# coqui-ai/TTS

Measured on NVIDIA H100. Metric: audio_samples_per_sec, higher is better.
Workload: dtype f32

## Files before the change

### tts_b200/csrc/conv_tc.cuh

```cuda
#pragma once
#include <cuda_runtime.h>
#include <stdint.h>

namespace b200tts {
namespace tc {

enum : int { PREC_FP32 = 0, PREC_BF16 = 1, PREC_FP16 = 2, PREC_F16X3 = 4 };
enum : int { ERR_RANGE = 1 };
constexpr float F16X3_MAX = 65504.f;
constexpr uint32_t SPIN_LIMIT = 1u << 22;

__device__ __forceinline__ uint32_t smem_u32(const void* p) { return (uint32_t)__cvta_generic_to_shared(p); }

__device__ __forceinline__ void mbar_init(uint32_t bar, uint32_t count) {
    asm volatile("mbarrier.init.shared::cta.b64 [%0], %1;" ::"r"(bar), "r"(count));
}
__device__ __forceinline__ void mbar_arrive(uint32_t bar) {
    asm volatile("mbarrier.arrive.shared::cta.b64 _, [%0];" ::"r"(bar) : "memory");
}
__device__ __forceinline__ void mbar_expect_tx(uint32_t bar, uint32_t bytes) {
    asm volatile("mbarrier.arrive.expect_tx.shared::cta.b64 _, [%0], %1;" ::"r"(bar), "r"(bytes) : "memory");
}
__device__ __forceinline__ bool mbar_wait(uint32_t bar, uint32_t parity, int* err) {
#pragma unroll 1
    for (uint32_t i = 0; i < SPIN_LIMIT; ++i) {
        uint32_t ok;
        asm volatile("{\n.reg .pred p;\nmbarrier.try_wait.parity.shared::cta.b64 p, [%1], %2;\nselp.u32 %0, 1, 0, p;\n}"
                     : "=r"(ok) : "r"(bar), "r"(parity) : "memory");
        if (ok) return true;
    }
    if (err) { *reinterpret_cast<volatile int*>(err) = 1; __threadfence_system(); }
    return false;
}
__device__ __forceinline__ void bulk_g2s(uint32_t dst, const void* src, uint32_t bytes, uint32_t bar) {
    asm volatile("cp.async.bulk.shared::cluster.global.mbarrier::complete_tx::bytes [%0], [%1], %2, [%3];"
                 ::"r"(dst), "l"(src), "r"(bytes), "r"(bar) : "memory");
}
__device__ __forceinline__ void fence_async_smem() { asm volatile("fence.proxy.async.shared::cta;" ::: "memory"); }

__device__ __forceinline__ uint64_t make_desc(uint32_t saddr, uint32_t lbo_bytes) {
    uint64_t d = 0;
    d |= (uint64_t)((saddr >> 4) & 0x3FFF);
    d |= (uint64_t)((lbo_bytes >> 4) & 0x3FFF) << 16;
    d |= (uint64_t)((128u >> 4) & 0x3FFF) << 32;
    return d;
}

__device__ __forceinline__ void wgmma_fence() { asm volatile("wgmma.fence.sync.aligned;" ::: "memory"); }
__device__ __forceinline__ void wgmma_commit() { asm volatile("wgmma.commit_group.sync.aligned;" ::: "memory"); }
template <int N>
__device__ __forceinline__ void wgmma_wait() { asm volatile("wgmma.wait_group.sync.aligned %0;" ::"n"(N) : "memory"); }

#define B200_WGMMA_D128                                                                                                       \
    "{%0,%1,%2,%3,%4,%5,%6,%7,%8,%9,%10,%11,%12,%13,%14,%15,%16,%17,%18,%19,%20,%21,%22,%23,%24,%25,%26,%27,%28,%29,%30,%31,"    \
    "%32,%33,%34,%35,%36,%37,%38,%39,%40,%41,%42,%43,%44,%45,%46,%47,%48,%49,%50,%51,%52,%53,%54,%55,%56,%57,%58,%59,%60,%61,%62,%63," \
    "%64,%65,%66,%67,%68,%69,%70,%71,%72,%73,%74,%75,%76,%77,%78,%79,%80,%81,%82,%83,%84,%85,%86,%87,%88,%89,%90,%91,%92,%93,%94,%95," \
    "%96,%97,%98,%99,%100,%101,%102,%103,%104,%105,%106,%107,%108,%109,%110,%111,%112,%113,%114,%115,%116,%117,%118,%119,%120,%121,%122,%123,%124,%125,%126,%127},"
#define B200_WGMMA_D128_OPS(d)                                                                                                \
    "+f"(d[0]), "+f"(d[1]), "+f"(d[2]), "+f"(d[3]), "+f"(d[4]), "+f"(d[5]), "+f"(d[6]), "+f"(d[7]),                          \
    "+f"(d[8]), "+f"(d[9]), "+f"(d[10]), "+f"(d[11]), "+f"(d[12]), "+f"(d[13]), "+f"(d[14]), "+f"(d[15]),                    \
    "+f"(d[16]), "+f"(d[17]), "+f"(d[18]), "+f"(d[19]), "+f"(d[20]), "+f"(d[21]), "+f"(d[22]), "+f"(d[23]),                  \
    "+f"(d[24]), "+f"(d[25]), "+f"(d[26]), "+f"(d[27]), "+f"(d[28]), "+f"(d[29]), "+f"(d[30]), "+f"(d[31]),                  \
    "+f"(d[32]), "+f"(d[33]), "+f"(d[34]), "+f"(d[35]), "+f"(d[36]), "+f"(d[37]), "+f"(d[38]), "+f"(d[39]),                  \
    "+f"(d[40]), "+f"(d[41]), "+f"(d[42]), "+f"(d[43]), "+f"(d[44]), "+f"(d[45]), "+f"(d[46]), "+f"(d[47]),                  \
    "+f"(d[48]), "+f"(d[49]), "+f"(d[50]), "+f"(d[51]), "+f"(d[52]), "+f"(d[53]), "+f"(d[54]), "+f"(d[55]),                  \
    "+f"(d[56]), "+f"(d[57]), "+f"(d[58]), "+f"(d[59]), "+f"(d[60]), "+f"(d[61]), "+f"(d[62]), "+f"(d[63]),                  \
    "+f"(d[64]), "+f"(d[65]), "+f"(d[66]), "+f"(d[67]), "+f"(d[68]), "+f"(d[69]), "+f"(d[70]), "+f"(d[71]),                  \
    "+f"(d[72]), "+f"(d[73]), "+f"(d[74]), "+f"(d[75]), "+f"(d[76]), "+f"(d[77]), "+f"(d[78]), "+f"(d[79]),                  \
    "+f"(d[80]), "+f"(d[81]), "+f"(d[82]), "+f"(d[83]), "+f"(d[84]), "+f"(d[85]), "+f"(d[86]), "+f"(d[87]),                  \
    "+f"(d[88]), "+f"(d[89]), "+f"(d[90]), "+f"(d[91]), "+f"(d[92]), "+f"(d[93]), "+f"(d[94]), "+f"(d[95]),                  \
    "+f"(d[96]), "+f"(d[97]), "+f"(d[98]), "+f"(d[99]), "+f"(d[100]), "+f"(d[101]), "+f"(d[102]), "+f"(d[103]),              \
    "+f"(d[104]), "+f"(d[105]), "+f"(d[106]), "+f"(d[107]), "+f"(d[108]), "+f"(d[109]), "+f"(d[110]), "+f"(d[111]),          \
    "+f"(d[112]), "+f"(d[113]), "+f"(d[114]), "+f"(d[115]), "+f"(d[116]), "+f"(d[117]), "+f"(d[118]), "+f"(d[119]),          \
    "+f"(d[120]), "+f"(d[121]), "+f"(d[122]), "+f"(d[123]), "+f"(d[124]), "+f"(d[125]), "+f"(d[126]), "+f"(d[127])

__device__ __forceinline__ void wgmma_tf32_m64n256(float* d, uint64_t adesc, uint64_t bdesc, uint32_t acc) {
    asm volatile(
        "{\n.reg .pred p;\nsetp.ne.b32 p, %130, 0;\n"
        "wgmma.mma_async.sync.aligned.m64n256k8.f32.tf32.tf32 " B200_WGMMA_D128
        " %128, %129, p, 1, 1;\n}"
        : B200_WGMMA_D128_OPS(d)
        : "l"(adesc), "l"(bdesc), "r"(acc)
        : "memory");
}

__device__ __forceinline__ void wgmma_bf16_m64n256(float* d, uint64_t adesc, uint64_t bdesc, uint32_t acc) {
    asm volatile(
        "{\n.reg .pred p;\nsetp.ne.b32 p, %130, 0;\n"
        "wgmma.mma_async.sync.aligned.m64n256k16.f32.bf16.bf16 " B200_WGMMA_D128
        " %128, %129, p, 1, 1, 0, 0;\n}"
        : B200_WGMMA_D128_OPS(d)
        : "l"(adesc), "l"(bdesc), "r"(acc)
        : "memory");
}
__device__ __forceinline__ void wgmma_f16_m64n256(float* d, uint64_t adesc, uint64_t bdesc, uint32_t acc) {
    asm volatile(
        "{\n.reg .pred p;\nsetp.ne.b32 p, %130, 0;\n"
        "wgmma.mma_async.sync.aligned.m64n256k16.f32.f16.f16 " B200_WGMMA_D128
        " %128, %129, p, 1, 1, 0, 0;\n}"
        : B200_WGMMA_D128_OPS(d)
        : "l"(adesc), "l"(bdesc), "r"(acc)
        : "memory");
}
__device__ __forceinline__ void wgmma_f16_m64n256_rs(float* d, const uint32_t (&a)[4], uint64_t bdesc, uint32_t acc) {
    asm volatile(
        "{\n.reg .pred p;\nsetp.ne.b32 p, %133, 0;\n"
        "wgmma.mma_async.sync.aligned.m64n256k16.f32.f16.f16 " B200_WGMMA_D128
        " {%128, %129, %130, %131}, %132, p, 1, 1, 0;\n}"
        : B200_WGMMA_D128_OPS(d)
        : "r"(a[0]), "r"(a[1]), "r"(a[2]), "r"(a[3]), "l"(bdesc), "r"(acc)
        : "memory");
}

__device__ __forceinline__ void ldsm_x4(uint32_t (&r)[4], uint32_t addr) {
    asm volatile("ldmatrix.sync.aligned.m8n8.x4.shared.b16 {%0, %1, %2, %3}, [%4];"
                 : "=r"(r[0]), "=r"(r[1]), "=r"(r[2]), "=r"(r[3]) : "r"(addr) : "memory");
}
__device__ __forceinline__ uint32_t f16x2_times_2m11(uint32_t v) {
    uint32_t r;
    asm("mul.rn.f16x2 %0, %1, %2;" : "=r"(r) : "r"(v), "r"(0x10001000u));
    return r;
}

__device__ __forceinline__ uint32_t cvt_bf16x2(float lo, float hi) {
    uint32_t r;
    asm("cvt.rn.bf16x2.f32 %0, %1, %2;" : "=r"(r) : "f"(hi), "f"(lo));
    return r;
}
__device__ __forceinline__ uint32_t cvt_f16x2(float lo, float hi) {
    uint32_t r;
    asm("cvt.rn.f16x2.f32 %0, %1, %2;" : "=r"(r) : "f"(hi), "f"(lo));
    return r;
}
__device__ __forceinline__ void split_f16x2(float a, float b, uint32_t& hi, uint32_t& lo) {
    hi = cvt_f16x2(a, b);
    float ha, hb;
    asm("{\n.reg .b16 l, h;\nmov.b32 {l, h}, %2;\ncvt.f32.f16 %0, l;\ncvt.f32.f16 %1, h;\n}" : "=f"(ha), "=f"(hb) : "r"(hi));
    lo = cvt_f16x2((a - ha) * 2048.f, (b - hb) * 2048.f);
}

}
}
```

### tts_b200/csrc/conv_tc3.cuh

```cuda
#pragma once
#include <cuda_runtime.h>
#include <stdint.h>

#include "conv_tc.cuh"

namespace b200tts {
namespace tc3 {

using namespace tc;

constexpr int TT2 = 256;
constexpr int MROWS = 128;
constexpr int KC2 = 8;
constexpr int KC16 = 16;
constexpr int RAWS = 324;
constexpr int NRAW = 3;
constexpr int NA2 = 2;
constexpr int NB2 = 3;
constexpr int ACC_LD = 260;
constexpr int ACC_BYTES = MROWS * ACC_LD * 4;
constexpr int NPW = 3;
constexpr int NPROD = 32 * NPW;
constexpr int NCONS = 256;
constexpr int W_PROD = 8, W_LOAD = 8 + NPW;
constexpr int NTHREADS2 = 32 * (W_LOAD + 1);

struct Tc3Args {
    const float* x; long long x_bs; int x_cs; int Tin;
    float in_slope;
    const void* w;
    const float* rscale;
    const float* bias;
    const float* cond; long long cond_bs;
    int Cin, K, dil, pad, Rows, N;
    float* y; long long y_bs; int y_cs; int Tout;
    int ups;
    int Tq;
    const float* res; long long res_bs; int res_cs;
    const float* ymask; long long ymask_bs;
    float scale; float post_div; int relu; int accum; int mask_post;
    int mask_pre;
    int gate;
    int split;
    float* y2; long long y2_bs; int y2_cs; int accum2;
    int KJ;
    int dil_blk;
    int tstep;
    int rows_pad;
    int raw_w;
    int B, n_ttiles, n_rtiles;
    int* err;
    const int* lens; int rate_q, need_q, rate_in, need_in;
    int pref_off;
    int q_lo, q_hi, in_lo, t_lo;
    int near_src; float near_scale;
    const float* film; long long film_bs; int film_cs, film_half;
    const float* act_add; int lrelu; float act_param;
};

__device__ __forceinline__ int near_col(int t, int src, int dst, float scale) {
    if (dst == src) return t;
    if (dst == 2 * src) return t >> 1;
    return min((int)floorf(__fmul_rn((float)t, scale)), src - 1);
}

static inline size_t smem_bytes3(int rows_pad, int prec = PREC_FP32) {
    const bool b16 = prec == PREC_BF16 || prec == PREC_FP16;
    const size_t raw_ch = b16 ? KC16 : KC2, nsl = b16 ? 2 : 4;
    return (size_t)NRAW * raw_ch * RAWS * 4 + (size_t)NA2 * (nsl * rows_pad * 16) + NB2 * (nsl * MROWS * 16) + ACC_BYTES + 512;
}
static inline size_t ragged_table_bytes(int B) { return ((size_t)(B + 1) * sizeof(int) + 15) / 16 * 16; }

__device__ __forceinline__ void cp_async16(uint32_t dst, const void* src) {
    asm volatile("cp.async.cg.shared.global [%0], [%1], 16;" ::"r"(dst), "l"(src) : "memory");
}
__device__ __forceinline__ void cp_async16_zfill(uint32_t dst, const void* src, uint32_t src_bytes) {
    asm volatile("cp.async.cg.shared.global [%0], [%1], 16, %2;" ::"r"(dst), "l"(src), "r"(src_bytes) : "memory");
}
__device__ __forceinline__ void cp_async4_zfill(uint32_t dst, const void* src, uint32_t src_bytes) {
    asm volatile("cp.async.ca.shared.global [%0], [%1], 4, %2;" ::"r"(dst), "l"(src), "r"(src_bytes) : "memory");
}
__device__ __forceinline__ void named_bar_sync(int id, int n) { asm volatile("bar.sync %0, %1;" ::"r"(id), "r"(n) : "memory"); }
__device__ __forceinline__ void acc_ld16(const float* p, float* v) {
#pragma unroll
    for (int j = 0; j < 4; ++j) {
        const float4 t = *reinterpret_cast<const float4*>(p + 4 * j);
        v[4 * j] = t.x; v[4 * j + 1] = t.y; v[4 * j + 2] = t.z; v[4 * j + 3] = t.w;
    }
}

constexpr int TSTEP_GROUPED = 240;

template <bool HR, bool HA, bool SC>
__device__ __forceinline__ void lean_tile(const float* at, const float* bias, const float* rscale, const float* cond, int lane,
                                          const float* rq, float* yq, long long rcs, long long ycs, int row0, int Rows,
                                          bool do_st) {
    const int r8 = lane & 7, p4 = lane >> 3;
    const float* rrow[4];
    float* yrow[4];
    bool st_ok[4];
    float bv[4], sv[4];
#pragma unroll
    for (int i = 0; i < 4; ++i) {
        const int ri = row0 + 8 * i + r8, rci = ri < Rows ? ri : Rows - 1;
        rrow[i] = rq + (long long)rci * rcs + 4 * p4;
        yrow[i] = yq + (long long)rci * ycs + 4 * p4;
        st_ok[i] = do_st && ri < Rows;
        bv[i] = bias[rci];
        if (cond) bv[i] += __ldg(cond + rci);
        sv[i] = SC ? rscale[rci] : 1.f;
    }
    const float* ap = at + r8 * ACC_LD + 4 * p4;
    float r0[16], r1[16];
    auto pf = [&](int cg, float* r_) {
        if constexpr (HR) {
#pragma unroll
            for (int i = 0; i < 4; ++i)
                asm volatile("ld.global.v4.f32 {%0,%1,%2,%3}, [%4];" : "=f"(r_[4 * i]), "=f"(r_[4 * i + 1]), "=f"(r_[4 * i + 2]), "=f"(r_[4 * i + 3]) : "l"(rrow[i] + cg));
        }
    };
    auto group = [&](int cg, const float* rv, float* rn) {
        float o[16];
        if (cg + 16 < 128) pf(cg + 16, rn);
        if constexpr (HA) {
#pragma unroll
            for (int i = 0; i < 4; ++i)
                asm volatile("ld.global.v4.f32 {%0,%1,%2,%3}, [%4];" : "=f"(o[4 * i]), "=f"(o[4 * i + 1]), "=f"(o[4 * i + 2]), "=f"(o[4 * i + 3]) : "l"(yrow[i] + cg));
        }
#pragma unroll
        for (int i = 0; i < 4; ++i) {
            float4 t = *reinterpret_cast<const float4*>(ap + 8 * i * ACC_LD + cg);
            if constexpr (SC) { t.x *= sv[i]; t.y *= sv[i]; t.z *= sv[i]; t.w *= sv[i]; }
            t.x += bv[i]; t.y += bv[i]; t.z += bv[i]; t.w += bv[i];
            if constexpr (HR) { t.x += rv[4 * i]; t.y += rv[4 * i + 1]; t.z += rv[4 * i + 2]; t.w += rv[4 * i + 3]; }
            if constexpr (HA) { t.x += o[4 * i]; t.y += o[4 * i + 1]; t.z += o[4 * i + 2]; t.w += o[4 * i + 3]; }
            if (st_ok[i]) *reinterpret_cast<float4*>(yrow[i] + cg) = t;
        }
    };
    pf(0, r0);
#pragma unroll 1
    for (int cg = 0; cg < 128; cg += 32) {
        group(cg, r0, r1);
        group(cg + 16, r1, r0);
    }
}

template <bool SC, bool WG = false>
__device__ __forceinline__ void general_tile_body(const Tc3Args& a, const float* arow, int b, int rt, int q0, int lq, int half,
                                                  int lane) {
    const int ups = a.ups;
    const int r = rt * MROWS + lq * 32 + lane;
    const bool rok = r < a.Rows;
    const int rc = rok ? r : a.Rows - 1;
    const int qb = q0 + half * 128;
    float bias = a.bias[rc];
    if (a.cond) bias += __ldg(a.cond + (long long)b * a.cond_bs + rc);
    const float rs = SC ? a.rscale[rc] : 1.f;
    auto acc_ld = [&](const float* p, float* v) {
        acc_ld16(p, v);
        if constexpr (SC) {
#pragma unroll
            for (int i = 0; i < 16; ++i) v[i] *= rs;
        }
    };
    if constexpr (WG) {
        if (!rok) return;
        const long long rcs = (long long)rc;
        float* yrow = a.y + (long long)b * a.y_bs + rcs * a.y_cs;
        float* y2row = a.y2 ? a.y2 + (long long)b * a.y2_bs + rcs * a.y2_cs : nullptr;
        const float* rrow = a.res ? a.res + (long long)b * a.res_bs + rcs * a.res_cs : nullptr;
        const float* srow = a.film ? a.film + (long long)b * a.film_bs + rcs * a.film_cs : nullptr;
        const float* crow = srow ? srow + (long long)a.film_half * a.film_cs : nullptr;
        const float add = a.act_add ? __ldg(a.act_add + b) : 0.f;
        const bool has_add = a.act_add != nullptr, lrelu = a.lrelu != 0;
        const float slope = a.act_param;
        const bool vec_ok = ((reinterpret_cast<uintptr_t>(yrow) | reinterpret_cast<uintptr_t>(y2row) |
                              reinterpret_cast<uintptr_t>(rrow) | reinterpret_cast<uintptr_t>(srow) |
                              reinterpret_cast<uintptr_t>(crow)) & 15) == 0;
        for (int cg = 0; cg < 128; cg += 16) {
            float v[16];
            acc_ld(arow + cg, v);
#pragma unroll
            for (int j = 0; j < 4; ++j) {
                const int qq = qb + cg + 4 * j;
                if (qq >= a.Tout) break;
                const bool vec = vec_ok && qq + 3 < a.Tout;
                float r4[4] = {0.f, 0.f, 0.f, 0.f}, s4[4] = {0.f, 0.f, 0.f, 0.f}, c4[4] = {1.f, 1.f, 1.f, 1.f};
                if (vec) {
                    if (rrow) { const float4 t = *reinterpret_cast<const float4*>(rrow + qq); r4[0] = t.x; r4[1] = t.y; r4[2] = t.z; r4[3] = t.w; }
                    if (srow) {
                        const float4 t = *reinterpret_cast<const float4*>(srow + qq); s4[0] = t.x; s4[1] = t.y; s4[2] = t.z; s4[3] = t.w;
                        const float4 u = *reinterpret_cast<const float4*>(crow + qq); c4[0] = u.x; c4[1] = u.y; c4[2] = u.z; c4[3] = u.w;
                    }
                } else {
#pragma unroll
                    for (int e = 0; e < 4; ++e) {
                        const int qe = min(qq + e, a.Tout - 1);
                        if (rrow) r4[e] = rrow[qe];
                        if (srow) { s4[e] = srow[qe]; c4[e] = crow[qe]; }
                    }
                }
                float o[4], p[4];
#pragma unroll
                for (int e = 0; e < 4; ++e) {
                    float u = __fadd_rn(v[4 * j + e], bias);
                    if (lrelu) u = u > 0.f ? u : __fmul_rn(u, slope);
                    if (has_add) u = __fadd_rn(u, add);
                    if (rrow) u = __fadd_rn(u, r4[e]);
                    p[e] = u;
                    o[e] = srow ? __fadd_rn(s4[e], __fmul_rn(c4[e], u)) : u;
                }
                if (vec) {
                    if (y2row) *reinterpret_cast<float4*>(y2row + qq) = make_float4(p[0], p[1], p[2], p[3]);
                    *reinterpret_cast<float4*>(yrow + qq) = make_float4(o[0], o[1], o[2], o[3]);
                } else {
#pragma unroll
                    for (int e = 0; e < 4; ++e)
                        if (qq + e < a.Tout) {
                            if (y2row) y2row[qq + e] = p[e];
                            yrow[qq + e] = o[e];
                        }
                }
            }
        }
        return;
    }
    if (a.gate) {
        float* yrow = a.y + (long long)b * a.y_bs + (long long)(rc >> 1) * a.y_cs;
        const bool vec_ok = ((a.y_cs & 3) == 0) && ((reinterpret_cast<uintptr_t>(yrow) & 15) == 0);
        const bool even = (lane & 1) == 0;
        for (int cg = 0; cg < 128; cg += 16) {
            float v[16];
            acc_ld(arow + cg, v);
            const int q = qb + cg;
#pragma unroll
            for (int i = 0; i < 16; ++i) {
                const float u = v[i] + bias;
                const float act = even ? tanhf(u) : 1.f / (1.f + expf(-u));
                const float other = __shfl_xor_sync(0xffffffffu, act, 1);
                v[i] = act * other;
            }
            if (rok && even) {
#pragma unroll
                for (int j = 0; j < 4; ++j) {
                    const int qq = q + 4 * j;
                    if (vec_ok && qq + 3 < a.Tout) *reinterpret_cast<float4*>(yrow + qq) = make_float4(v[4 * j], v[4 * j + 1], v[4 * j + 2], v[4 * j + 3]);
                    else {
#pragma unroll
                        for (int e = 0; e < 4; ++e) if (qq + e < a.Tout) yrow[qq + e] = v[4 * j + e];
                    }
                }
            }
        }
    } else if (ups == 1) {
        float* yrow = a.y + (long long)b * a.y_bs + (long long)rc * a.y_cs;
        bool acc_r = a.accum != 0, mpost_r = a.mask_post != 0;
        if (a.split > 0) {
            if (rc < a.split) { acc_r = true; mpost_r = true; }
            else { yrow = a.y2 + (long long)b * a.y2_bs + (long long)(rc - a.split) * a.y2_cs; acc_r = a.accum2 != 0; mpost_r = false; }
        }
        const float* rrow = a.res ? a.res + (long long)b * a.res_bs + (long long)rc * a.res_cs : nullptr;
        const float* mrow = a.ymask ? a.ymask + (long long)b * a.ymask_bs : nullptr;
        const int ycs_eff = (a.split > 0 && rc >= a.split) ? a.y2_cs : a.y_cs;
        const bool vec_ok = ((ycs_eff & 3) == 0) && (!a.res || (a.res_cs & 3) == 0) &&
                            ((reinterpret_cast<uintptr_t>(yrow) & 15) == 0) &&
                            (!rrow || (reinterpret_cast<uintptr_t>(rrow) & 15) == 0);
        float rA[16], oA[16], rB[16], oB[16];
        auto prefetch = [&](int cg, float* r_, float* o_) {
            const int q = qb + cg;
#pragma unroll
            for (int j = 0; j < 4; ++j) {
                const int qq = q + 4 * j;
                if (vec_ok && qq + 3 < a.Tout) {
                    if (rrow) asm volatile("ld.global.v4.f32 {%0,%1,%2,%3}, [%4];" : "=f"(r_[4 * j]), "=f"(r_[4 * j + 1]), "=f"(r_[4 * j + 2]), "=f"(r_[4 * j + 3]) : "l"(rrow + qq));
                    if (acc_r) asm volatile("ld.global.v4.f32 {%0,%1,%2,%3}, [%4];" : "=f"(o_[4 * j]), "=f"(o_[4 * j + 1]), "=f"(o_[4 * j + 2]), "=f"(o_[4 * j + 3]) : "l"(yrow + qq));
                } else {
#pragma unroll
                    for (int e = 0; e < 4; ++e) {
                        const int qe = min(qq + e, a.Tout - 1);
                        if (rrow) asm volatile("ld.global.f32 %0, [%1];" : "=f"(r_[4 * j + e]) : "l"(rrow + qe));
                        if (acc_r) asm volatile("ld.global.f32 %0, [%1];" : "=f"(o_[4 * j + e]) : "l"(yrow + qe));
                    }
                }
            }
        };
        auto group = [&](int cg, const float* rv, const float* ov, float* rn, float* on) {
            float v[16];
            if (rok && cg + 16 < 128) prefetch(cg + 16, rn, on);
            acc_ld(arow + cg, v);
            const int q = qb + cg;
#pragma unroll
            for (int i = 0; i < 16; ++i) {
                float u = v[i] + bias;
                if (a.relu) u = fmaxf(u, 0.f);
                const float mk = mrow ? __ldg(mrow + min(q + i, a.Tout - 1)) : 1.f;
                if (a.mask_pre) u *= mk;
                if (a.res) u += rv[i];
                u *= a.scale;
                if (acc_r) u += ov[i];
                if (a.post_div != 1.f) u = u / a.post_div;
                if (mpost_r) u *= mk;
                v[i] = u;
            }
            if (rok) {
#pragma unroll
                for (int j = 0; j < 4; ++j) {
                    const int qq = q + 4 * j;
                    if (vec_ok && qq + 3 < a.Tout) {
                        *reinterpret_cast<float4*>(yrow + qq) = make_float4(v[4 * j], v[4 * j + 1], v[4 * j + 2], v[4 * j + 3]);
                    } else {
#pragma unroll
                        for (int e = 0; e < 4; ++e) if (qq + e < a.Tout) yrow[qq + e] = v[4 * j + e];
                    }
                }
            }
        };
        if (rok) prefetch(0, rA, oA);
#pragma unroll 1
        for (int cg = 0; cg < 128; cg += 32) {
            group(cg, rA, oA, rB, oB);
            group(cg + 16, rB, oB, rA, oA);
        }
    } else {
        if (!rok) return;
        const int co = rc / ups, ph = rc - co * ups;
        float* yrow = a.y + (long long)b * a.y_bs + (long long)co * a.y_cs + ph;
        for (int cg = 0; cg < 128; cg += 16) {
            float v[16];
            acc_ld(arow + cg, v);
#pragma unroll
            for (int i = 0; i < 16; ++i) {
                const int q = qb + cg + i;
                float u = v[i] + bias;
                if (a.relu) u = fmaxf(u, 0.f);
                const long long t = (long long)q * ups;
                if (q < a.Tq && t + ph < a.Tout) yrow[t] = u;
            }
        }
    }
}

template <bool SC>
__device__ __noinline__ void general_tile_call(const Tc3Args& a_ref, const float* arow, int b, int rt, int q0, int lq, int half,
                                               int lane) {
    const Tc3Args a = a_ref;
    general_tile_body<SC>(a, arow, b, rt, q0, lq, half, lane);
}

template <int GRP, bool SC>
__device__ __forceinline__ void grouped_tile(const Tc3Args& a, const float* accs, int b, int q0, int lq, int half, int lane) {
    constexpr int CH = 128 / GRP;
    constexpr int NQ = CH / 32;
    constexpr int NV = 4 * NQ;
    const int tq = lq * 32 + lane;
    const int co = (tq * NQ) >> 2;
    const int coff = 4 * ((tq & (4 / NQ - 1)) * NQ);
    const int cbeg = half ? 128 : 0;
    const int cend = half ? a.tstep : min(128, a.tstep);
    const bool has_res = a.res != nullptr, acc_r = a.accum != 0;
    const bool vec_ok = ((a.y_cs & 3) == 0) && ((a.y_bs & 3) == 0) && ((reinterpret_cast<uintptr_t>(a.y) & 15) == 0) &&
                        (!a.res || (((a.res_cs & 3) == 0) && ((a.res_bs & 3) == 0) && ((reinterpret_cast<uintptr_t>(a.res) & 15) == 0)));
    const bool fast = vec_ok && (q0 + a.tstep <= a.Tout);
    const float* rrow = has_res ? a.res + (long long)b * a.res_bs + (long long)co * a.res_cs : nullptr;
    float* yrow = a.y + (long long)b * a.y_bs + (long long)co * a.y_cs;
    float bias = a.bias[co];
    if (a.cond) bias += __ldg(a.cond + (long long)b * a.cond_bs + co);
    const float rs = SC ? a.rscale[co] : 1.f;
    auto load = [&](const float* rr, int q, float* dst) {
#pragma unroll
        for (int j = 0; j < NQ; ++j) {
            const int qq = q + 4 * j;
            if (fast || (vec_ok && qq + 3 < a.Tout)) {
                const float4 t = *reinterpret_cast<const float4*>(rr + qq);
                dst[4 * j] = t.x; dst[4 * j + 1] = t.y; dst[4 * j + 2] = t.z; dst[4 * j + 3] = t.w;
            } else {
#pragma unroll
                for (int e = 0; e < 4; ++e) dst[4 * j + e] = rr[min(qq + e, a.Tout - 1)];
            }
        }
    };
#pragma unroll 1
    for (int cg = cbeg; cg < cend; cg += 16) {
        float R[NV], rv[NV], ov[NV];
        if (has_res) load(rrow, q0 + cg + coff, rv);
        if (acc_r) load(yrow, q0 + cg + coff, ov);
        const float* p = accs + co * ACC_LD + cg + coff;
#pragma unroll
        for (int i = 0; i < NV; ++i) {
            const float p0 = p[i], p1 = p[CH * ACC_LD + a.dil + i];
            float s = p0 + p1;
            if constexpr (GRP == 4) s += p[2 * CH * ACC_LD + 2 * a.dil + i] + p[3 * CH * ACC_LD + 3 * a.dil + i];
            if constexpr (SC) s *= rs;
            R[i] = s;
        }
#pragma unroll
        for (int i = 0; i < NV; ++i) {
            float u = R[i] + bias;
            if (a.relu) u = fmaxf(u, 0.f);
            if (has_res) u += rv[i];
            u *= a.scale;
            if (acc_r) u += ov[i];
            if (a.post_div != 1.f) u = u / a.post_div;
            R[i] = u;
        }
        const int q = q0 + cg + coff;
#pragma unroll
        for (int j = 0; j < NQ; ++j) {
            const int qq = q + 4 * j;
            if (fast || (vec_ok && qq + 3 < a.Tout)) {
                *reinterpret_cast<float4*>(yrow + qq) = make_float4(R[4 * j], R[4 * j + 1], R[4 * j + 2], R[4 * j + 3]);
            } else {
#pragma unroll
                for (int e = 0; e < 4; ++e) if (qq + e < a.Tout) yrow[qq + e] = R[4 * j + e];
            }
        }
    }
}

template <int GRP, bool LEAN = true, int PREC = PREC_FP32, bool REFL = false, bool NEAR = false, bool WG = false>
__device__ __forceinline__ void tc3_body(const Tc3Args& a) {
    extern __shared__ __align__(128) unsigned char smem[];
    constexpr bool X3 = PREC == PREC_F16X3;
    constexpr bool B16 = PREC == PREC_BF16 || PREC == PREC_FP16;
    constexpr int KCH = PREC != PREC_FP32 ? KC16 : KC2;
    constexpr int RCH = B16 ? KC16 : KC2;
    constexpr int SPC = KCH / RCH;
    constexpr int NSL = B16 ? 2 : 4;
    constexpr int SLC = PREC != PREC_FP32 ? 8 : 4;
    constexpr int NB = NB2;
    constexpr bool SC = X3;
    const int tid = threadIdx.x, warp = tid >> 5, lane = tid & 31;
    const int ROWS = a.rows_pad, RAWW = a.raw_w, K = a.KJ;
    const uint32_t rawStage = (uint32_t)RCH * RAWS * 4;
    const uint32_t slabA = (uint32_t)ROWS * 16, stageA = NSL * slabA;
    const uint32_t slabB = (uint32_t)MROWS * 16, stageB = NSL * slabB;
    unsigned char* smRaw = smem;
    unsigned char* smA = smRaw + NRAW * rawStage;
    unsigned char* smB = smA + NA2 * stageA;
    float* accs = reinterpret_cast<float*>(smB + NB * stageB);
    uint64_t* bars = reinterpret_cast<uint64_t*>(reinterpret_cast<unsigned char*>(accs) + ACC_BYTES);
    const int A_FULL = 0, A_EMPTY = NA2, B_FULL = 2 * NA2, B_EMPTY = 2 * NA2 + NB;
    const uint32_t bar0 = smem_u32(bars);
    auto BAR = [&](int i) { return bar0 + 8u * (uint32_t)i; };

    const int nchunks = (a.Cin + KCH - 1) / KCH;
    const bool ragged = a.lens != nullptr;
    int* pref = reinterpret_cast<int*>(smem + a.pref_off);
    if (ragged) {
        for (int b = tid; b < a.B; b += NTHREADS2) {
            const long long e = (long long)a.lens[b] * a.rate_q + a.need_q;
            const int ext = (int)(e < (long long)a.Tq ? (e > 0 ? e : 0) : (long long)a.Tq);
            const int t_hi = (min(ext, a.q_hi) + a.tstep - 1) / a.tstep;
            pref[b + 1] = max(0, t_hi - a.t_lo) * a.n_rtiles;
        }
        __syncthreads();
        if (warp == 0) {
            const int per = (a.B + 31) / 32, lo = lane * per, hi = min(a.B, lo + per);
            int sum = 0;
            for (int b = lo; b < hi; ++b) sum += pref[b + 1];
            int incl = sum;
#pragma unroll
            for (int o = 1; o < 32; o <<= 1) { const int n = __shfl_up_sync(0xffffffffu, incl, o); if (lane >= o) incl += n; }
            int run = incl - sum;
            for (int b = lo; b < hi; ++b) { const int c = pref[b + 1]; pref[b + 1] = run + c; run += c; }
            if (lane == 0) pref[0] = 0;
        }
        __syncthreads();
    }
    const int tiles_total = ragged ? pref[a.B] : a.B * a.n_rtiles * a.n_ttiles;
    const int my_tiles = (tiles_total > (int)blockIdx.x) ? (tiles_total - 1 - (int)blockIdx.x) / (int)gridDim.x + 1 : 0;

    if (tid == 0) {
        for (int i = 0; i < NA2; ++i) { mbar_init(BAR(A_FULL + i), NPW); mbar_init(BAR(A_EMPTY + i), NCONS / 32); }
        for (int i = 0; i < NB; ++i) { mbar_init(BAR(B_FULL + i), 1); mbar_init(BAR(B_EMPTY + i), NCONS / 32); }
        asm volatile("fence.mbarrier_init.release.cluster;" ::: "memory");
    }
    __syncthreads();
    asm volatile("griddepcontrol.launch_dependents;" ::: "memory");
    if (warp != W_LOAD) asm volatile("griddepcontrol.wait;" ::: "memory");

    auto decode = [&](int it, int& b, int& rt, int& q0) {
        const int tile = (int)blockIdx.x + it * (int)gridDim.x;
        if (ragged) {
            int lo = 0, hi = a.B;
            while (hi - lo > 1) { const int mid = (lo + hi) >> 1; if (pref[mid] <= tile) lo = mid; else hi = mid; }
            b = lo;
            const int local = tile - pref[b], nt = (pref[b + 1] - pref[b]) / a.n_rtiles;
            rt = local / nt;
            q0 = (a.t_lo + local - rt * nt) * a.tstep;
            return;
        }
        const int tt = tile % a.n_ttiles, rest = tile / a.n_ttiles;
        rt = rest % a.n_rtiles;
        b = rest / a.n_rtiles;
        q0 = (a.t_lo + tt) * a.tstep;
    };
    auto input_extent = [&](int b) -> int {
        if (!ragged) return a.Tin;
        const long long e = (long long)a.lens[b] * a.rate_in + a.need_in;
        return (int)(e < (long long)a.Tin ? (e > 0 ? e : 0) : (long long)a.Tin);
    };

    if (warp >= W_PROD && warp < W_PROD + NPW) {
        const int ptid = tid - 32 * W_PROD;
        const int total = my_tiles * nchunks * SPC;
        const int vec_per_row = RAWW / 4;
        const int nvec = KC2 * vec_per_row;
        const float slope = a.in_slope;
        const float* const xg = a.x;
        const long long x_bs = a.x_bs;
        const int x_cs = a.x_cs, Cin = a.Cin, pad = a.pad;
        bool ok = true;
        constexpr int NIT = X3 ? 1 : 2;
        constexpr int MAXV = (8 * 81 + NPROD - 1) / NPROD, MAXI = (NIT * 320 + NPROD - 1) / NPROD;
        int v_ch[MAXV], v_t[MAXV], v_src[MAXV];
        uint32_t v_dst[MAXV];
#pragma unroll
        for (int e = 0; e < MAXV; ++e) {
            const int v = ptid + e * NPROD;
            const int ch = v / vec_per_row, j = v - ch * vec_per_row;
            v_ch[e] = (v < nvec) ? ch : -1;
            v_t[e] = 4 * j;
            v_src[e] = ch * x_cs + 4 * j;
            v_dst[e] = (uint32_t)(ch * RAWS + 4 * j) * 4u;
        }
        int i_raw[MAXI], i_dst[MAXI];
#pragma unroll
        for (int e = 0; e < MAXI; ++e) {
            const int idx = ptid + e * NPROD;
            const int sl = idx / ROWS, r = idx - sl * ROWS;
            i_raw[e] = (idx < NIT * ROWS) ? (SLC * sl) * RAWS + r : -1;
            i_dst[e] = (int)(sl * slabA) + r * 16;
        }
        int iss_it = 0, iss_c = 0, iss_h = 0, iss_ring = 0, iss_tal = 0, iss_Tin = 0;
        const float* iss_row = xg;
        bool iss_new = true, iss_int = false;
        int tr_it = 0, tr_c = 0, tr_h = 0, tr_ring = 0, tr_q0 = 0, as = 0;
        uint32_t pa_empty = 1;
        bool tr_new = true;
        const uint32_t raw_u32 = smem_u32(smRaw);
        float amax = 0.f;
        auto issue = [&](int g) {
            if (g < total) {
                if (iss_new) {
                    int b_, rt_, q0_;
                    decode(iss_it, b_, rt_, q0_);
                    iss_Tin = input_extent(b_);
                    iss_tal = (q0_ - pad) & ~3;
                    iss_row = xg + (long long)b_ * x_bs;
                    iss_int = !NEAR && iss_tal >= (a.in_lo & ~3) && iss_tal + RAWW <= iss_Tin && (Cin & (KCH - 1)) == 0;
                    iss_new = false;
                }
                const int ch0 = iss_c * KCH + iss_h * RCH;
#pragma unroll
                for (int h = 0; h < RCH / KC2; ++h) {
                    const uint32_t dst0 = raw_u32 + (uint32_t)iss_ring * rawStage + (uint32_t)(h * KC2 * RAWS * 4);
                    if (iss_int) {
                        const float* src = iss_row + (long long)(ch0 + h * KC2) * x_cs + iss_tal;
#pragma unroll
                        for (int e = 0; e < MAXV; ++e)
                            if (v_ch[e] >= 0) cp_async16(dst0 + v_dst[e], src + v_src[e]);
                    } else {
#pragma unroll
                        for (int e = 0; e < MAXV; ++e) {
                            if (v_ch[e] < 0) continue;
                            const int t = iss_tal + v_t[e];
                            const int cg = ch0 + h * KC2 + v_ch[e];
                            if constexpr (NEAR) {
                                const float* rowp = iss_row + (long long)(cg < Cin ? cg : 0) * x_cs;
#pragma unroll
                                for (int q = 0; q < 4; ++q) {
                                    const int tt = t + q;
                                    const bool in = cg < Cin && tt >= 0 && tt < iss_Tin;
                                    const int src = in ? near_col(tt, a.near_src, iss_Tin, a.near_scale) : 0;
                                    cp_async4_zfill(dst0 + v_dst[e] + 4u * q, rowp + src, in ? 4u : 0u);
                                }
                                continue;
                            }
                            if (REFL && (t < 0 || t + 4 > iss_Tin)) {
                                const float* rowp = iss_row + (long long)(cg < Cin ? cg : 0) * x_cs;
#pragma unroll
                                for (int q = 0; q < 4; ++q) {
                                    int tt = t + q;
                                    tt = tt < 0 ? -tt : (tt >= iss_Tin ? 2 * iss_Tin - 2 - tt : tt);
                                    const bool in = cg < Cin && tt >= 0 && tt < iss_Tin;
                                    cp_async4_zfill(dst0 + v_dst[e] + 4u * q, rowp + (in ? tt : 0), in ? 4u : 0u);
                                }
                                continue;
                            }
                            int nb = 0;
                            if (cg < Cin && t >= (a.in_lo & ~3)) nb = 4 * max(0, min(4, iss_Tin - t));
                            const int tsafe = (t >= 0 && t < iss_Tin) ? t : 0;
                            const float* src = iss_row + (long long)(cg < Cin ? cg : 0) * x_cs + tsafe;
                            cp_async16_zfill(dst0 + v_dst[e], src, (uint32_t)nb);
                        }
                    }
                }
                if (++iss_h == SPC) { iss_h = 0; if (++iss_c == nchunks) { iss_c = 0; ++iss_it; iss_new = true; } }
            }
            if (++iss_ring == NRAW) iss_ring = 0;
            asm volatile("cp.async.commit_group;" ::: "memory");
        };
        for (int g = 0; g < NRAW - 1; ++g) issue(g);
        for (int g = 0; g < total && ok; ++g) {
            asm volatile("cp.async.wait_group %0;" ::"n"(NRAW - 2) : "memory");
            named_bar_sync(1, NPROD);
            issue(g + NRAW - 1);
            if (tr_h == 0 && g >= NA2 * SPC) ok = mbar_wait(BAR(A_EMPTY + as), pa_empty, a.err);
            if (!ok) break;
            if (tr_new) {
                int b_, rt_;
                decode(tr_it, b_, rt_, tr_q0);
                tr_new = false;
            }
            const int tin0 = tr_q0 - pad, off = tin0 - (tin0 & ~3);
            const float* raw = reinterpret_cast<const float*>(smRaw + tr_ring * rawStage) + off;
            unsigned char* base = smA + as * stageA;
            float u[MAXI][SLC];
#pragma unroll
            for (int e = 0; e < MAXI; ++e) {
                const float* rp = raw + (i_raw[e] < 0 ? 0 : i_raw[e]);
#pragma unroll
                for (int i = 0; i < SLC; ++i) u[e][i] = rp[i * RAWS];
            }
            if constexpr (X3) {
#pragma unroll
                for (int e = 0; e < MAXI; ++e) {
                    if (i_raw[e] < 0) continue;
                    uint32_t ph[4], pl[4];
#pragma unroll
                    for (int i = 0; i < 4; ++i) {
                        const float w0 = fmaxf(u[e][2 * i], u[e][2 * i] * slope);
                        const float w1 = fmaxf(u[e][2 * i + 1], u[e][2 * i + 1] * slope);
                        amax = fmaxf(amax, fmaxf(fabsf(w0), fabsf(w1)));
                        split_f16x2(w0, w1, ph[i], pl[i]);
                    }
                    *reinterpret_cast<uint4*>(base + tr_h * slabA + i_dst[e]) = make_uint4(ph[0], ph[1], ph[2], ph[3]);
                    *reinterpret_cast<uint4*>(base + (2 + tr_h) * slabA + i_dst[e]) = make_uint4(pl[0], pl[1], pl[2], pl[3]);
                }
            } else if constexpr (B16) {
#pragma unroll
                for (int e = 0; e < MAXI; ++e) {
                    if (i_raw[e] < 0) continue;
                    uint32_t p[4];
#pragma unroll
                    for (int i = 0; i < 4; ++i) {
                        const float w0 = fmaxf(u[e][2 * i], u[e][2 * i] * slope);
                        const float w1 = fmaxf(u[e][2 * i + 1], u[e][2 * i + 1] * slope);
                        p[i] = PREC == PREC_BF16 ? cvt_bf16x2(w0, w1) : cvt_f16x2(w0, w1);
                    }
                    *reinterpret_cast<uint4*>(base + i_dst[e]) = make_uint4(p[0], p[1], p[2], p[3]);
                }
            } else {
#pragma unroll
                for (int e = 0; e < MAXI; ++e) {
                    if (i_raw[e] < 0) continue;
                    float4 hi, lo;
                    float* ph = &hi.x; float* pl = &lo.x;
#pragma unroll
                    for (int i = 0; i < 4; ++i) {
                        const float w_ = fmaxf(u[e][i], u[e][i] * slope);
                        const float h = __uint_as_float(__float_as_uint(w_) & 0xFFFFE000u);
                        ph[i] = h;
                        pl[i] = w_ - h;
                    }
                    *reinterpret_cast<float4*>(base + i_dst[e]) = hi;
                    *reinterpret_cast<float4*>(base + 2 * slabA + i_dst[e]) = lo;
                }
            }
            if (++tr_ring == NRAW) tr_ring = 0;
            if (++tr_h < SPC) continue;
            tr_h = 0;
            fence_async_smem();
            __syncwarp();
            if (lane == 0) mbar_arrive(BAR(A_FULL + as));
            if (++tr_c == nchunks) { tr_c = 0; ++tr_it; tr_new = true; }
            if (++as == NA2) { as = 0; pa_empty ^= 1u; }
        }
        asm volatile("cp.async.wait_group 0;" ::: "memory");
        if (X3 && amax >= F16X3_MAX && a.err) { *reinterpret_cast<volatile int*>(a.err + ERR_RANGE) = 1; __threadfence_system(); }
    } else if (warp == W_LOAD) {
        if (lane < NB) {
            const int total = nchunks * K;
            const long long all = (long long)my_tiles * total;
            const uint32_t full = BAR(B_FULL + lane), empty = BAR(B_EMPTY + lane);
            const uint32_t dst = smem_u32(smB + lane * stageB);
            int it = 0, j = lane;
            while (j >= total && it < my_tiles) { j -= total; ++it; }
            int cur_it = -1;
            const unsigned char* wsrc = nullptr;
            uint32_t par = 1;
            bool ok = true, first = true;
            for (long long gi = lane; gi < all && ok; gi += NB) {
                if (it != cur_it) {
                    int b_, rt, q0_;
                    decode(it, b_, rt, q0_);
                    wsrc = reinterpret_cast<const unsigned char*>(a.w) + (size_t)rt * total * stageB;
                    cur_it = it;
                }
                if (!first) { ok = mbar_wait(empty, par, a.err); if (!ok) break; }
                mbar_expect_tx(full, stageB);
                bulk_g2s(dst, wsrc + (size_t)j * stageB, stageB, full);
                first = false;
                par ^= 1u;
                j += NB;
                while (j >= total) { j -= total; ++it; }
            }
        }
        __syncwarp();
    } else if (warp < W_PROD) {
        const int wg = warp >> 2, lq = warp & 3, half = warp >> 2;
        const uint64_t wdesc0 = make_desc(smem_u32(smB) + (uint32_t)wg * 64 * 16, slabB);
        const uint64_t wlo_off = (uint64_t)((2 * slabB) >> 4), wslot = (uint64_t)(stageB >> 4);
        const uint32_t whi_lds = smem_u32(smB) + (uint32_t)(lane >> 4) * slabB + (uint32_t)(warp * 16 + (lane & 15)) * 16;
        const uint64_t xstep = (uint64_t)a.dil_blk;
        bool ok = true;
        int sa = 0; uint32_t pa = 0;
        int sb = 0; uint32_t pb = 0;
        float* const st_row = accs + (wg * 64 + lq * 16 + (lane >> 2)) * ACC_LD + 2 * (lane & 3);
#pragma unroll 1
        for (int it = 0; it < my_tiles; ++it) {
            float d[128];
#pragma unroll
            for (int i = 0; i < 128; ++i) d[i] = 0.f;
            uint32_t acc = 0u;
            int rel_b = -1, rel_a = -1;
            auto release = [&]() {
                __syncwarp();
                if (lane == 0) {
                    if (rel_b >= 0) mbar_arrive(BAR(B_EMPTY + rel_b));
                    if (rel_a >= 0) mbar_arrive(BAR(A_EMPTY + rel_a));
                }
            };
#pragma unroll 1
            for (int c = 0; c < nchunks; ++c) {
                if (ok) ok = mbar_wait(BAR(A_FULL + sa), pa, a.err);
                const uint32_t abase = smem_u32(smA + sa * stageA);
                uint64_t xh = make_desc(abase, slabA), xl = make_desc(abase + 2 * slabA, slabA);
#pragma unroll 1
                for (int k = 0; k < K; ++k) {
                    if (ok) ok = mbar_wait(BAR(B_FULL + sb), pb, a.err);
                    if (ok) {
                        const uint64_t w_hi = wdesc0 + (uint64_t)sb * wslot, w_lo = w_hi + wlo_off;
                        uint32_t whs[4];
                        if constexpr (X3) {
                            ldsm_x4(whs, whi_lds + (uint32_t)sb * stageB);
#pragma unroll
                            for (int i = 0; i < 4; ++i) whs[i] = f16x2_times_2m11(whs[i]);
                        }
                        wgmma_fence();
                        if constexpr (PREC == PREC_BF16) {
                            wgmma_bf16_m64n256(d, w_hi, xh, acc);
                        } else if constexpr (PREC == PREC_FP16) {
                            wgmma_f16_m64n256(d, w_hi, xh, acc);
                        } else if constexpr (X3) {
                            wgmma_f16_m64n256_rs(d, whs, xl, acc);
                            wgmma_commit();
                            wgmma_f16_m64n256(d, w_lo, xh, 1u);
                            wgmma_f16_m64n256(d, w_hi, xh, 1u);
                        } else {
                            wgmma_tf32_m64n256(d, w_hi, xl, acc);
                            wgmma_tf32_m64n256(d, w_lo, xh, 1u);
                            wgmma_tf32_m64n256(d, w_hi, xh, 1u);
                        }
                        wgmma_commit();
                    }
                    wgmma_wait<1>();
                    release();
                    rel_b = sb;
                    rel_a = (k == K - 1) ? sa : -1;
                    acc = 1u;
                    xh += xstep; xl += xstep;
                    if (++sb == NB) { sb = 0; pb ^= 1u; }
                }
                if (++sa == NA2) { sa = 0; pa ^= 1u; }
            }
            wgmma_wait<0>();
            release();
            named_bar_sync(4, NCONS);
#pragma unroll
            for (int j = 0; j < 32; ++j) {
                *reinterpret_cast<float2*>(st_row + 8 * j) = make_float2(d[4 * j], d[4 * j + 1]);
                *reinterpret_cast<float2*>(st_row + 8 * ACC_LD + 8 * j) = make_float2(d[4 * j + 2], d[4 * j + 3]);
            }
            named_bar_sync(4, NCONS);
            if (!ok) continue;
            int b, rt, q0;
            decode(it, b, rt, q0);
            if constexpr (GRP > 1) {
                grouped_tile<GRP, SC>(a, accs, b, q0, lq, half, lane);
            } else {
                const int qb = q0 + half * 128;
                const float* at = accs + lq * 32 * ACC_LD + half * 128;
                const bool lean = LEAN && a.ups == 1 && !a.gate && a.split == 0 && !a.relu && !a.ymask && a.scale == 1.f &&
                                  a.post_div == 1.f && qb + 128 <= a.Tout &&
                                  ((a.y_cs & 3) == 0) && ((a.y_bs & 3) == 0) && ((reinterpret_cast<uintptr_t>(a.y) & 15) == 0) &&
                                  (!a.res || (((a.res_cs & 3) == 0) && ((a.res_bs & 3) == 0) && ((reinterpret_cast<uintptr_t>(a.res) & 15) == 0)));
                if (lean) {
                    const int row0 = rt * MROWS + lq * 32;
                    const float* cond = a.cond ? a.cond + (long long)b * a.cond_bs : nullptr;
                    float* yq = a.y + (long long)b * a.y_bs + qb;
                    const bool hres = a.res != nullptr, hacc = a.accum != 0;
                    const float* rq = hres ? a.res + (long long)b * a.res_bs + qb : yq;
                    if (hres) { if (hacc) lean_tile<true, true, SC>(at, a.bias, a.rscale, cond, lane, rq, yq, a.res_cs, a.y_cs, row0, a.Rows, true);
                                else lean_tile<true, false, SC>(at, a.bias, a.rscale, cond, lane, rq, yq, a.res_cs, a.y_cs, row0, a.Rows, true); }
                    else { if (hacc) lean_tile<false, true, SC>(at, a.bias, a.rscale, cond, lane, rq, yq, 0, a.y_cs, row0, a.Rows, true);
                           else lean_tile<false, false, SC>(at, a.bias, a.rscale, cond, lane, rq, yq, 0, a.y_cs, row0, a.Rows, true); }
                } else if constexpr (LEAN) {
                    general_tile_call<SC>(a, at + lane * ACC_LD, b, rt, q0, lq, half, lane);
                } else {
                    general_tile_body<SC, WG>(a, at + lane * ACC_LD, b, rt, q0, lq, half, lane);
                }
            }
        }
    }
}

template <int PREC, bool REFL = false>
__global__ void __launch_bounds__(NTHREADS2, 1) conv1d_tc3_kernel(const __grid_constant__ Tc3Args a) { tc3_body<1, true, PREC, REFL>(a); }
template <int PREC>
__global__ void __launch_bounds__(NTHREADS2, 1) conv1d_tc3x_kernel(const __grid_constant__ Tc3Args a) { tc3_body<1, false, PREC>(a); }
template <int GRP, int PREC, bool REFL = false>
__global__ void __launch_bounds__(NTHREADS2, 1) conv1d_tc3g_kernel(const __grid_constant__ Tc3Args a) { tc3_body<GRP, true, PREC, REFL>(a); }

template <int PREC, bool NEAR>
__global__ void __launch_bounds__(NTHREADS2, 1) conv1d_tc3w_kernel(const __grid_constant__ Tc3Args a) {
    tc3_body<1, false, PREC, false, NEAR, true>(a);
}

typedef void (*Tc3Kernel)(const Tc3Args);
static inline Tc3Kernel wavegrad_kernel(int prec, bool near) {
    if (prec == PREC_F16X3) return near ? conv1d_tc3w_kernel<PREC_F16X3, true> : conv1d_tc3w_kernel<PREC_F16X3, false>;
    if (prec == PREC_FP32) return near ? conv1d_tc3w_kernel<PREC_FP32, true> : conv1d_tc3w_kernel<PREC_FP32, false>;
    return nullptr;
}
static inline Tc3Kernel plain_kernel(int prec, bool lean, bool reflect = false) {
    if (reflect) {
        if (prec == PREC_BF16) return conv1d_tc3_kernel<PREC_BF16, true>;
        if (prec == PREC_FP16) return conv1d_tc3_kernel<PREC_FP16, true>;
        if (prec == PREC_F16X3) return conv1d_tc3_kernel<PREC_F16X3, true>;
        return conv1d_tc3_kernel<PREC_FP32, true>;
    }
    if (prec == PREC_BF16) return lean ? conv1d_tc3_kernel<PREC_BF16> : conv1d_tc3x_kernel<PREC_BF16>;
    if (prec == PREC_FP16) return lean ? conv1d_tc3_kernel<PREC_FP16> : conv1d_tc3x_kernel<PREC_FP16>;
    if (prec == PREC_F16X3) return lean ? conv1d_tc3_kernel<PREC_F16X3> : conv1d_tc3x_kernel<PREC_F16X3>;
    return lean ? conv1d_tc3_kernel<PREC_FP32> : conv1d_tc3x_kernel<PREC_FP32>;
}
template <bool REFL>
static inline Tc3Kernel grouped_kernel_t(int grp, int prec) {
    if (prec == PREC_BF16) return grp == 2 ? conv1d_tc3g_kernel<2, PREC_BF16, REFL> : conv1d_tc3g_kernel<4, PREC_BF16, REFL>;
    if (prec == PREC_FP16) return grp == 2 ? conv1d_tc3g_kernel<2, PREC_FP16, REFL> : conv1d_tc3g_kernel<4, PREC_FP16, REFL>;
    if (prec == PREC_F16X3) return grp == 2 ? conv1d_tc3g_kernel<2, PREC_F16X3, REFL> : conv1d_tc3g_kernel<4, PREC_F16X3, REFL>;
    return grp == 2 ? conv1d_tc3g_kernel<2, PREC_FP32, REFL> : conv1d_tc3g_kernel<4, PREC_FP32, REFL>;
}
static inline Tc3Kernel grouped_kernel(int grp, int prec = PREC_FP32, bool reflect = false) {
    return reflect ? grouped_kernel_t<true>(grp, prec) : grouped_kernel_t<false>(grp, prec);
}

}
}
```

Measured before the change: 31.02 million.

## Use TMA bulk copies for residual prefetch and output store in lean epilogue

```diff
diff --git a/tts_b200/csrc/conv_tc.cuh b/tts_b200/csrc/conv_tc.cuh
--- a/tts_b200/csrc/conv_tc.cuh
+++ b/tts_b200/csrc/conv_tc.cuh
@@ -36,6 +36,12 @@
     asm volatile("cp.async.bulk.shared::cluster.global.mbarrier::complete_tx::bytes [%0], [%1], %2, [%3];"
                  ::"r"(dst), "l"(src), "r"(bytes), "r"(bar) : "memory");
 }
+__device__ __forceinline__ void bulk_s2g(void* dst, uint32_t src, uint32_t bytes) {
+    asm volatile("cp.async.bulk.global.shared::cta.bulk_group [%0], [%1], %2;" ::"l"(dst), "r"(src), "r"(bytes) : "memory");
+}
+__device__ __forceinline__ void bulk_commit() { asm volatile("cp.async.bulk.commit_group;" ::: "memory"); }
+__device__ __forceinline__ void bulk_wait_read() { asm volatile("cp.async.bulk.wait_group.read 0;" ::: "memory"); }
+__device__ __forceinline__ void bulk_wait_all() { asm volatile("cp.async.bulk.wait_group 0;" ::: "memory"); }
 __device__ __forceinline__ void fence_async_smem() { asm volatile("fence.proxy.async.shared::cta;" ::: "memory"); }
 
 __device__ __forceinline__ uint64_t make_desc(uint32_t saddr, uint32_t lbo_bytes) {
diff --git a/tts_b200/csrc/conv_tc3.cuh b/tts_b200/csrc/conv_tc3.cuh
--- a/tts_b200/csrc/conv_tc3.cuh
+++ b/tts_b200/csrc/conv_tc3.cuh
@@ -145,6 +145,22 @@
     }
 }
 
+template <bool HR, bool SC>
+__device__ __forceinline__ void bulk_combine(const float* d, float* st_row, const float (&bv)[2], const float (&sv)[2]) {
+#pragma unroll
+    for (int j = 0; j < 32; ++j) {
+#pragma unroll
+        for (int h = 0; h < 2; ++h) {
+            float2* p = reinterpret_cast<float2*>(st_row + h * 8 * ACC_LD + 8 * j);
+            float2 t = make_float2(d[4 * j + 2 * h], d[4 * j + 2 * h + 1]);
+            if constexpr (SC) { t.x *= sv[h]; t.y *= sv[h]; }
+            t.x += bv[h]; t.y += bv[h];
+            if constexpr (HR) { const float2 r = *p; t.x += r.x; t.y += r.y; }
+            *p = t;
+        }
+    }
+}
+
 template <bool SC, bool WG = false>
 __device__ __forceinline__ void general_tile_body(const Tc3Args& a, const float* arow, int b, int rt, int q0, int lq, int half,
                                                   int lane) {
@@ -429,6 +445,7 @@
     constexpr int SLC = PREC != PREC_FP32 ? 8 : 4;
     constexpr int NB = NB2;
     constexpr bool SC = X3;
+    constexpr bool BULK = GRP == 1 && LEAN;
     const int tid = threadIdx.x, warp = tid >> 5, lane = tid & 31;
     const int ROWS = a.rows_pad, RAWW = a.raw_w, K = a.KJ;
     const uint32_t rawStage = (uint32_t)RCH * RAWS * 4;
@@ -439,7 +456,7 @@
     unsigned char* smB = smA + NA2 * stageA;
     float* accs = reinterpret_cast<float*>(smB + NB * stageB);
     uint64_t* bars = reinterpret_cast<uint64_t*>(reinterpret_cast<unsigned char*>(accs) + ACC_BYTES);
-    const int A_FULL = 0, A_EMPTY = NA2, B_FULL = 2 * NA2, B_EMPTY = 2 * NA2 + NB;
+    const int A_FULL = 0, A_EMPTY = NA2, B_FULL = 2 * NA2, B_EMPTY = 2 * NA2 + NB, RES_FULL = 2 * NA2 + 2 * NB;
     const uint32_t bar0 = smem_u32(bars);
     auto BAR = [&](int i) { return bar0 + 8u * (uint32_t)i; };
 
@@ -473,6 +490,7 @@
     if (tid == 0) {
         for (int i = 0; i < NA2; ++i) { mbar_init(BAR(A_FULL + i), NPW); mbar_init(BAR(A_EMPTY + i), NCONS / 32); }
         for (int i = 0; i < NB; ++i) { mbar_init(BAR(B_FULL + i), 1); mbar_init(BAR(B_EMPTY + i), NCONS / 32); }
+        for (int i = 0; i < NCONS / 32; ++i) mbar_init(BAR(RES_FULL + i), 1);
         asm volatile("fence.mbarrier_init.release.cluster;" ::: "memory");
     }
     __syncthreads();
@@ -718,8 +736,35 @@
         int sa = 0; uint32_t pa = 0;
         int sb = 0; uint32_t pb = 0;
         float* const st_row = accs + (wg * 64 + lq * 16 + (lane >> 2)) * ACC_LD + 2 * (lane & 3);
+        const int row_w = wg * 64 + lq * 16;
+        const bool bulk_layer = BULK && a.ups == 1 && !a.gate && a.split == 0 && !a.relu && !a.ymask &&
+                                a.scale == 1.f && a.post_div == 1.f && a.accum == 0 &&
+                                ((a.y_cs & 3) == 0) && ((a.y_bs & 3) == 0) && ((reinterpret_cast<uintptr_t>(a.y) & 15) == 0) &&
+                                (!a.res || (((a.res_cs & 3) == 0) && ((a.res_bs & 3) == 0) && ((reinterpret_cast<uintptr_t>(a.res) & 15) == 0)));
+        uint32_t pr = 0;
+        bool shared_epi = false;
 #pragma unroll 1
         for (int it = 0; it < my_tiles; ++it) {
+            bool bulk, pre;
+            {
+                int b, rt, q0;
+                decode(it, b, rt, q0);
+                const int nrows = min(16, a.Rows - (rt * MROWS + row_w));
+                bulk = bulk_layer && q0 + TT2 <= a.Tout;
+                pre = bulk && a.res != nullptr && nrows > 0;
+                if (bulk) {
+                    if (shared_epi) { fence_async_smem(); named_bar_sync(4, NCONS); }
+                    if (lane == 0) bulk_wait_read();
+                    __syncwarp();
+                }
+                if (pre && lane == 0) {
+                    const uint32_t rf = BAR(RES_FULL + warp);
+                    const float* src = a.res + (long long)b * a.res_bs + (long long)(rt * MROWS + row_w) * a.res_cs + q0;
+                    mbar_expect_tx(rf, (uint32_t)nrows * TT2 * 4);
+                    for (int r = 0; r < nrows; ++r)
+                        bulk_g2s(smem_u32(accs + (row_w + r) * ACC_LD), src + (long long)r * a.res_cs, TT2 * 4, rf);
+                }
+            }
             float d[128];
 #pragma unroll
             for (int i = 0; i < 128; ++i) d[i] = 0.f;
@@ -777,6 +822,42 @@
             }
             wgmma_wait<0>();
             release();
+            int b, rt, q0;
+            decode(it, b, rt, q0);
+            if (bulk) {
+                if (pre) {
+                    const bool landed = mbar_wait(BAR(RES_FULL + warp), pr, a.err);
+                    ok = ok && landed;
+                    pr ^= 1u;
+                }
+                shared_epi = false;
+                if (!ok) continue;
+                const int r0 = rt * MROWS + row_w, rl = r0 + (lane >> 2);
+                float bv[2], sv[2];
+#pragma unroll
+                for (int h = 0; h < 2; ++h) {
+                    const int rc = min(rl + 8 * h, a.Rows - 1);
+                    bv[h] = a.bias[rc];
+                    if (a.cond) bv[h] += __ldg(a.cond + (long long)b * a.cond_bs + rc);
+                    sv[h] = SC ? a.rscale[rc] : 1.f;
+                }
+                if (pre) bulk_combine<true, SC>(d, st_row, bv, sv);
+                else bulk_combine<false, SC>(d, st_row, bv, sv);
+                fence_async_smem();
+                __syncwarp();
+                if (lane == 0) {
+                    const int nrows = min(16, a.Rows - r0);
+                    float* dst = a.y + (long long)b * a.y_bs + (long long)r0 * a.y_cs + q0;
+                    for (int r = 0; r < nrows; ++r)
+                        bulk_s2g(dst + (long long)r * a.y_cs, smem_u32(accs + (row_w + r) * ACC_LD), TT2 * 4);
+                    bulk_commit();
+                }
+                continue;
+            }
+            if constexpr (BULK) {
+                if (lane == 0) bulk_wait_read();
+                __syncwarp();
+            }
             named_bar_sync(4, NCONS);
 #pragma unroll
             for (int j = 0; j < 32; ++j) {
@@ -784,9 +865,8 @@
                 *reinterpret_cast<float2*>(st_row + 8 * ACC_LD + 8 * j) = make_float2(d[4 * j + 2], d[4 * j + 3]);
             }
             named_bar_sync(4, NCONS);
+            shared_epi = true;
             if (!ok) continue;
-            int b, rt, q0;
-            decode(it, b, rt, q0);
             if constexpr (GRP > 1) {
                 grouped_tile<GRP, SC>(a, accs, b, q0, lq, half, lane);
             } else {
@@ -813,6 +893,10 @@
                 }
             }
         }
+        if constexpr (BULK) {
+            if (lane == 0) bulk_wait_all();
+            __syncwarp();
+        }
     }
 }
 
```

Result: faster. 32.53 million, median of 6 (+4.9%).
